# awslabs/dgl-ke

Hardware: AMD Instinct MI355X
Metric: positive edges/sec (whole node) (higher is better)
Workload: dtype f32

## Files before the change

dgl-ke_amd/csrc/kge_common.hpp:

```cpp
#pragma once
#include <hip/hip_runtime.h>
#include <stdint.h>
#include "../../include/kge_hip.h"

#define KGE_WAVE 64
#define KGE_BLOCK 256
#define KGE_WAVES_PER_BLOCK (KGE_BLOCK / KGE_WAVE)

typedef float f32x4 __attribute__((ext_vector_type(4)));
#define MFMA16(a, b, c) __builtin_amdgcn_mfma_f32_16x16x4f32((a), (b), (c), 0, 0, 0)

#ifdef KGE_TIMELINE
#define KGE_TL_PER_KERNEL 8192
static __device__ unsigned long long *kge_tl_buf = nullptr;
__device__ __forceinline__ void kge_tl_mark(int kid, int n) {
    asm volatile("s_waitcnt vmcnt(0) lgkmcnt(0)" ::: "memory");
    const int wid = (int)(blockIdx.x * (blockDim.x >> 6) + (threadIdx.x >> 6));
    if ((threadIdx.x & 63) == 0 && kge_tl_buf && wid < KGE_TL_PER_KERNEL)
        kge_tl_buf[((size_t)kid * KGE_TL_PER_KERNEL + wid) * 8 + 4 + n] = wall_clock64();
}
struct KgeTlScope {
    unsigned long long t0; int kid; int wid;
    __device__ __forceinline__ KgeTlScope(int kid_, int wid_) : kid(kid_), wid(wid_) { t0 = wall_clock64(); }
    __device__ __forceinline__ void mark(int n) { kge_tl_mark(kid, n); }
// ... 152 lines not shown
__device__ __forceinline__ float sgnf(float x) { return (x > 0.f) ? 1.f : ((x < 0.f) ? -1.f : 0.f); }

__device__ __forceinline__ float reg_grad3(float x, float coef) { return 3.f * coef * x * fabsf(x); }
__device__ __forceinline__ float reg_val3(float x) { const float ax = fabsf(x); return ax * ax * ax; }
__device__ __forceinline__ float reg_grad(float x, float coef, int q) {
    if (__builtin_constant_p(q) && q == 3) return reg_grad3(x, coef);
    const float ax = fabsf(x);
    const float pw = __builtin_amdgcn_exp2f((float)(q - 1) * __builtin_amdgcn_logf(ax));
    return ax > 0.f ? copysignf(coef * (float)q * pw, x) : 0.f;
}
__device__ __forceinline__ float reg_val(float x, int q) {
    if (__builtin_constant_p(q) && q == 3) return reg_val3(x);
    const float ax = fabsf(x);
    return ax > 0.f ? __builtin_amdgcn_exp2f((float)q * __builtin_amdgcn_logf(ax)) : 0.f;
}

__device__ __forceinline__ float reg_acc(float rv, float x, int q) {
    if (__builtin_constant_p(q) && q == 3) { const float ax = fabsf(x); return fmaf(ax * ax, ax, rv); }
    return rv + reg_val(x, q);
}

__device__ __forceinline__ float sigmoidf_(float x) {
    if (x >= 0.f) { return 1.f / (1.f + expf(-x)); }
    const float e = expf(x);
    return e / (1.f + e);
}
__device__ __forceinline__ float neg_logsigmoid(float z) {
    return fmaxf(-z, 0.f) + log1pf(expf(-fabsf(z)));
}

constexpr bool is_complex_model(int m) { return m == KGE_COMPLEX || m == KGE_ROTATE || m == KGE_SIMPLE; }
#define KGE_SIMPLE_CLAMP 20.f

__device__ __forceinline__ float fast_sigmoid(float x) { return __frcp_rn(1.f + __expf(-x)); }
__device__ __forceinline__ float fast_neg_logsigmoid(float z) {
    return fmaxf(-z, 0.f) + __logf(1.f + __expf(-fabsf(z)));
}
__device__ __forceinline__ void criterion_fast(int genre, float s, float label, float margin,
                                               float &val, float &dval) {
    if (genre == KGE_LOSS_HINGE) {
        const float v = margin - label * s;
        val = v < 0.f ? 0.f : v;
        dval = v < 0.f ? 0.f : -label;
    } else if (genre == KGE_LOSS_BCE) {
        val = label * fast_neg_logsigmoid(s) + (1.f - label) * fast_neg_logsigmoid(-s);
        dval = fast_sigmoid(s) - label;
    } else {
        const float z = label * s;
        val = fast_neg_logsigmoid(z);
        dval = -label * fast_sigmoid(-z);
    }
}

__device__ __forceinline__ void criterion(int genre, float s, float label, float margin,
                                          float &val, float &dval) {
    criterion_fast(genre, s, label, margin, val, dval);
}

__device__ __forceinline__ float mean_edge_weight(const float *w, int B, int lane, float pre = 0.f) {
    if (!w) return 1.f;
    if (pre > 0.f) return pre;
    float s = 0.f;
    for (int j = lane; j < B; j += KGE_WAVE) s += w[j];
    return wave_sum(s) / (float)B;
}

__device__ __forceinline__ int xcd_remap(int b, int nb) {
    const int q = nb >> 3, r = nb & 7, x = b & 7, k = b >> 3;
    return (x < r ? x * (q + 1) : r * (q + 1) + (x - r) * q) + k;
}

}

struct EdgeSrc {
    const float *hbase; const int64_t *hidx;
    const float *tbase; const int64_t *tidx;
    const float *rbase; const int64_t *ridx;
    kge::ShardMap em, rm;
};

struct LossParams {
    int genre, adv, pairwise;
    float adv_temp, margin;
// ... 60 lines not shown
    for (int r = 0; r < 8; ++r) pv[r] = *reinterpret_cast<const float4 *>(a.GNp + (int64_t)(r < nrw ? r : nrw - 1) * stride + 4 * t);
    float4 acc = pv[0];
#pragma unroll
    for (int r = 1; r < 8; ++r)
        if (r < nrw) { acc.x += pv[r].x; acc.y += pv[r].y; acc.z += pv[r].z; acc.w += pv[r].w; }
    for (int r = 8; r < nrw; ++r) {
        const float4 v = *reinterpret_cast<const float4 *>(a.GNp + r * stride + 4 * t);
        acc.x += v.x; acc.y += v.y; acc.z += v.z; acc.w += v.w;
    }
    if (a.reg_coef > 0.f && a.reg_norm > 0) {
        const int64_t j = (4 * t) / a.d_e;
        const int k = (int)((4 * t) % a.d_e);
        const float4 x = *reinterpret_cast<const float4 *>(kge::row_ptr(a.nbase, a.nidx, j, a.d_e) + k);
        acc.x += kge::reg_grad(x.x, a.reg_coef, a.reg_norm); acc.y += kge::reg_grad(x.y, a.reg_coef, a.reg_norm);
        acc.z += kge::reg_grad(x.z, a.reg_coef, a.reg_norm); acc.w += kge::reg_grad(x.w, a.reg_coef, a.reg_norm);
    }
    { kge::Pack<4> o; o.v[0] = acc.x; o.v[1] = acc.y; o.v[2] = acc.z; o.v[3] = acc.w; KGE_ST_NEXT<4>(a.GN + 4 * t, o); }
}

struct LossArgs {
    int B, N, genre, adv, pairwise;
    float adv_temp, margin;
    const float *pos, *neg, *w;
    float w_mean;
    float *dpos, *dneg;
    float *row_pos, *row_neg;
    float *acc;
    int l2_scale; float gamma;
    int l2_raw, l2_chunk; const float *asq, *bsq;
    float clampv;
    float *neg_copy;
    int skip_pos;
    int diag_chunk;
};

struct UpdateArgs {
    int model_d_e, d_r, UE, UR, reg_norm;
    float lr, eps, reg_coef;
    float *ent, *ent_state, *rel, *rel_state;
    kge::ShardMap em, rm;
    const int64_t *ue_id; const int32_t *ue_pos_ptr, *ue_pos_adj, *ue_neg_ptr, *ue_neg_slot;
    const int64_t *ur_id; const int32_t *ur_ptr, *ur_edge;
    const int32_t *ue_rec, *ur_rec;
    const int32_t *counts_dev;
    const float *GH, *GT, *GN, *GR;
    int transe_fast, neg_head; const float *P, *GA;
    const float *Q;
    float *reg_ent, *reg_rel;
    float *acc;
    float *g0, *gs0, *g1, *gs1, *gr, *gsr;
    int emit_ent, emit_rel;
    int emit_by_id;
    const int32_t *msg_rows;
    int msg_cap, msg_capT;
    int ld_e, ld_r;
    int32_t *rid;
    int ld_gs_e, ld_gs_r;
    int dry;
    const float *Hs, *Ts, *Rs;
    const float *Ns;
    int nd_chunk, nd_Ns, nd_Np;
    const float *GNp; int gn_parts; int64_t gn_stride; float gn_reg_coef; int gn_reg_norm;
    int ga_parts; int64_t ga_stride;
};
__device__ __forceinline__ int64_t gn_row(const UpdateArgs &a, int slot) {
    return a.nd_chunk ? (int64_t)(slot / a.nd_Ns) * a.nd_Np + a.nd_chunk + slot % a.nd_Ns : (int64_t)slot;
}
// ... 194 lines not shown
```

dgl-ke_amd/csrc/kge_loss_body.hpp:

```cpp
#pragma once
#include "kge_common.hpp"
#include "kge_update_body.hpp"

__device__ __forceinline__ void loss_args_lean(LossArgs &a) {
    a.genre = KGE_LOSS_LOGSIGMOID; a.pairwise = 0; a.skip_pos = 1; a.clampv = 0.f; a.neg_copy = nullptr;
    a.row_pos = nullptr; a.row_neg = nullptr; a.diag_chunk = 0;
}

template <int NPER>
__device__ __forceinline__ void loss_row_regs(const LossArgs &a, int64_t i, float (&nv)[NPER], float w, float p, int lane,
                                              int slot2) {
    using namespace kge;
    const int N = a.N;
    float *dn = a.dneg + i * (int64_t)N;
    float *cp = a.neg_copy ? a.neg_copy + i * (int64_t)N : nullptr;
    const int jd = a.diag_chunk > 0 ? (int)(i % a.diag_chunk) : -1;
    const float invB = 1.f / (float)a.B;
    const int slot = (int)(i & (KGE_ACC_SLOTS - 1));
    if (a.pairwise) {
        const float sc = w / ((float)a.B * (float)N);
        float lsum = 0.f, dsum = 0.f;
#pragma unroll
        for (int u = 0; u < NPER; ++u) {
            const int j = lane + 64 * u;
            if (j < N) {
                float val, dv;
                criterion_fast(a.genre, p - nv[u], 1.f, a.margin, val, dv);
                lsum += val * sc;
                const float dd = dv * sc;
                dsum += dd;
                if (cp) cp[j] = nv[u];
                float g = -dd;
                if (a.l2_scale) { const float d = a.gamma - nv[u]; g = d > 1e-15f ? g / d : 0.f; }
                if (a.clampv > 0.f && fabsf(nv[u]) >= a.clampv) g = 0.f;
                dn[j] = j == jd ? 0.f : g;
            }
        }
        lsum = wave_sum(lsum);
        dsum = wave_sum(dsum);
        if (lane == 0) {
            a.dpos[i] = (a.clampv > 0.f && fabsf(p) >= a.clampv) ? 0.f : dsum;
            if (a.row_pos) { a.row_pos[i] = 0.f; a.row_neg[i] = lsum; }
            if (a.acc) acc_add(&a.acc[2 * KGE_ACC_SLOTS + slot2], lsum, a.B <= KGE_ACC_SLOTS);
        }
        return;
    }
    float plw = 0.f;
    if (!a.skip_pos) {
        const float wm = mean_edge_weight(a.w, a.B, lane, a.w_mean);
        if (lane == 0) {
            float pl, dpl;
            criterion(a.genre, p, 1.f, a.margin, pl, dpl);
            a.dpos[i] = (a.clampv > 0.f && fabsf(p) >= a.clampv) ? 0.f : dpl * wm * 0.5f * invB;
            plw = pl * wm * invB;
            if (a.row_pos) a.row_pos[i] = plw;
        }
    }
    const float neg_label = a.genre == KGE_LOSS_BCE ? 0.f : -1.f;
    float mx = -INFINITY, Z = 1.f;
    float ex[NPER];
    if (a.adv) {
#pragma unroll
        for (int u = 0; u < NPER; ++u) if (lane + 64 * u < N) mx = fmaxf(mx, nv[u] * a.adv_temp);
        mx = wave_max(mx);
        float z = 0.f;
#pragma unroll
        for (int u = 0; u < NPER; ++u) {
            ex[u] = (lane + 64 * u < N) ? __expf(nv[u] * a.adv_temp - mx) : 0.f;
            z += ex[u];
        }
        Z = wave_sum(z);
    }
    const float invZ = 1.f / Z, invN = 1.f / (float)N;
    float acc = 0.f;
#pragma unroll
    for (int u = 0; u < NPER; ++u) {
        const int j = lane + 64 * u;
        if (j < N) {
            float nl, dnl;
            criterion_fast(a.genre, nv[u], neg_label, a.margin, nl, dnl);
            const float A = a.adv ? ex[u] * invZ : invN;
            acc += A * nl * w;
            float g = dnl * w * A * 0.5f * invB;
            if (cp) cp[j] = nv[u];
            if (a.l2_scale) { const float d = a.gamma - nv[u]; g = d > 1e-15f ? g / d : 0.f; }
            if (a.clampv > 0.f && fabsf(nv[u]) >= a.clampv) g = 0.f;
            dn[j] = j == jd ? 0.f : g;
        }
    }
    acc = wave_sum(acc) * invB;
    if (lane == 0) {
        if (a.row_neg) a.row_neg[i] = acc;
        if (a.acc) {
            const bool uq = a.B <= KGE_ACC_SLOTS;
            if (!a.skip_pos) acc_add(&a.acc[0 * KGE_ACC_SLOTS + slot], plw, uq);
            acc_add(&a.acc[1 * KGE_ACC_SLOTS + slot], acc, uq);
            acc_add(&a.acc[2 * KGE_ACC_SLOTS + slot2], 0.5f * (plw + acc), uq);
        }
    }
}
```

dgl-ke_amd/csrc/kge_neg_gemm.hip:

```cpp
#include "kge_common.hpp"
#include "kge_update_body.hpp"
#include "kge_edge_fwd_body.hpp"
#include "kge_sampler_tail.hpp"
#include "kge_loss_body.hpp"

using namespace kge;
KGE_TL_DEFINE(gemm)

#define KGE_PIN_ACC(x, y) do { asm volatile("" : "+a"(x), "+a"(y) :: "memory"); __builtin_amdgcn_sched_barrier(0); } while (0)
#define KGE_ORDER() do { asm volatile("" ::: "memory"); __builtin_amdgcn_sched_barrier(0); } while (0)

bool neg_mfma_supported(int model, int d_e, int N) {
    (void)N;
    if (model != KGE_TRANSE_L2 && model != KGE_DISTMULT && model != KGE_COMPLEX && model != KGE_SIMPLE &&
        model != KGE_RESCAL) return false;
    return d_e % 4 == 0;
}

bool neg_gemm_fused_loss_supported(int chunk, int N) { return N <= 256 && chunk <= 768; }

__device__ __forceinline__ float4 ldg4(const float *p) { return *reinterpret_cast<const float4 *>(p); }
__device__ __forceinline__ float4 zero4() { return make_float4(0.f, 0.f, 0.f, 0.f); }
__device__ __forceinline__ float sq4(const float4 &v) { return v.x * v.x + v.y * v.y + v.z * v.z + v.w * v.w; }

// ... 243 lines not shown
        float4 av[1], rv[1], bv[NB][1];
        av[0] = zero4(); rv[0] = zero4();
#pragma unroll
        for (int n = 0; n < NB; ++n) bv[n][0] = zero4();
        if (kfull * 16 + q * 4 < D) {
            av[0] = ldg4(Ap + kfull * 16);
            if (AM) rv[0] = ldg4(Rp + kfull * 16);
#pragma unroll
            for (int n = 0; n < NB; ++n) bv[n][0] = ldg4(Bp[n] + kfull * 16);
        }
        WF_MMA1(av, rv, bv, 0)
    }
#undef WF_LOAD
#undef WF_AFRAG
#undef WF_MMA1
#undef WF_MMA
#undef WF_MMA_G
#undef WF_PIN
#pragma unroll
    for (int n = 0; n < NB; ++n) {
        const int j = (jg * NB + n) * 16 + m;
#pragma unroll
        for (int r = 0; r < 4; ++r) {
            const int i = it * 16 + q * 4 + r;
            if (j < a.N && i < a.chunk) a.S[((int64_t)c * a.chunk + i) * a.N + j] = acc[n][0][r] + acc[n][1][r];
        }
    }
}

static inline int fwd_lds_stride(int D) { return ((D + 15) & ~15) + 4; }
static inline size_t fwd_lds_bytes(int D) { return (size_t)16 * fwd_lds_stride(D) * sizeof(float); }
static inline size_t fwd_lds_bytes_lf(int D) { return fwd_lds_bytes(D) + 32 * sizeof(float); }

template <int AM, bool LF = false, bool LLEAN = false>
__device__ __forceinline__ void neg_fwd_gemm_ldsa_body(const GemmArgs &a, int ti, int tj, int bid, int nblk, float *As,
                                                       const LossArgs *lap = nullptr, int *tickets = nullptr) {
    const int lane = threadIdx.x & 63, wv = threadIdx.x >> 6;
    const int tjg = (tj + 3) >> 2;
    int jg, sidx;
    const int nfull = (tj & 3) ? tjg - 1 : tjg, nheavy = a.C * ti * nfull;
    if (bid < nheavy) { const int L = xcd_remap(bid, nheavy); jg = L % nfull; sidx = L / nfull; }
    else { sidx = xcd_remap(bid - nheavy, nblk - nheavy); jg = tjg - 1; }
    const int it = sidx % ti, c = sidx / ti;
    const int jt = min(jg * 4 + wv, tj - 1);
    const bool tile_ok = jg * 4 + wv < tj;
    const int D = a.D, KP = ((D + 15) & ~15) + 4, n4 = D >> 2;
    const int m = lane & 15, q = lane >> 4;
    const int arow = threadIdx.x >> 4, ac = threadIdx.x & 15;
    const int64_t ie = (int64_t)c * a.chunk + min(it * 16 + arow, a.chunk - 1);
    const int64_t jl = (int64_t)c * a.N + min(jt * 16 + m, a.N - 1);
    const int64_t xid = a.xidx[ie], rid = a.ridx[ie];
    const int64_t jraw = *(a.nidx ? a.nidx + jl : a.xidx);
    const float *Xs = a.xbase + xid * D, *Rs = a.rbase + rid * D;
    const float *Bp = a.nbase + (a.nidx ? jraw : jl) * D + q * 4;
    float *Adst = As + arow * KP;
    const float *Ap = As + m * KP + q * 4;
    const float asg = a.asign;
    const int kfull = D >> 4;
    f32x4 acc0 = {0.f, 0.f, 0.f, 0.f}, acc1 = {0.f, 0.f, 0.f, 0.f};
    float4 a0[FU], b0[FU], a1[FU], b1[FU];
    float4 xv[8], rv[8];
    float asq_t = 0.f, bs0 = 0.f, bs1 = 0.f;
    if constexpr (AM == 3) {
        const int hd = D >> 1, h4 = hd >> 2;
        for (int c0 = 0; c0 < h4; c0 += 16 * 4) {
#pragma unroll
// ... 119 lines not shown
    } else {
        float bsq = 0.f;
        if constexpr (AM == 1) {
            bsq = bs0 + bs1;
            bsq += __shfl_xor(bsq, 16);
            bsq += __shfl_xor(bsq, 32);
        }
#pragma unroll
        for (int r = 0; r < 4; ++r) {
            const int i = it * 16 + q * 4 + r;
            float x = acc0[r] + acc1[r];
            if constexpr (AM == 1) x = a.gamma - sqrtf(fmaxf(fmaf(-2.f, x, Aq[q * 4 + r] + bsq), 1e-30f));
            if (j < a.N && i < a.chunk)
                __hip_atomic_store(a.S + ((int64_t)c * a.chunk + i) * a.N + j, x, __ATOMIC_RELAXED, __HIP_MEMORY_SCOPE_AGENT);
        }
    }
    }
    if constexpr (LF) {
        asm volatile("s_waitcnt vmcnt(0)" ::: "memory");
        __syncthreads();
        int *lastw = reinterpret_cast<int *>(Aq + 16);
        if (threadIdx.x == 0) {
            int *tk = tickets + (c * ti + it);
            const int old = __hip_atomic_fetch_add(tk, 1, __ATOMIC_RELAXED, __HIP_MEMORY_SCOPE_AGENT);
            const int last = old == tjg - 1;
            if (last) __hip_atomic_store(tk, 0, __ATOMIC_RELAXED, __HIP_MEMORY_SCOPE_AGENT);
            else if (old < 0 || old >= tjg) __builtin_trap();
            *lastw = last;
        }
        __syncthreads();
        if (!*lastw) return;
        LossArgs la = *lap;
        if constexpr (LLEAN) loss_args_lean(la);
        constexpr int NPER = 4;
        const int N = la.N;
        const int row0 = it * 16 + wv * 4;
        float nv[4][NPER];
#pragma unroll
        for (int r = 0; r < 4; ++r) {
            const int64_t gi = (int64_t)c * a.chunk + min(row0 + r, a.chunk - 1);
#pragma unroll
            for (int u = 0; u < NPER; ++u)
                nv[r][u] = __hip_atomic_load(a.S + gi * N + min(lane + 64 * u, N - 1), __ATOMIC_RELAXED, __HIP_MEMORY_SCOPE_AGENT);
        }
        float wr[4];
#pragma unroll
        for (int r = 0; r < 4; ++r) wr[r] = la.w ? la.w[(int64_t)c * a.chunk + min(row0 + r, a.chunk - 1)] : 1.f;
#pragma unroll
        for (int r = 0; r < 4; ++r) {
            if (row0 + r < a.chunk) {
                const int64_t gi = (int64_t)c * a.chunk + row0 + r;
#pragma unroll
                for (int u = 0; u < NPER; ++u) if (lane + 64 * u >= N) nv[r][u] = 0.f;
                loss_row_regs<NPER>(la, gi, nv[r], wr[r], 0.f, lane, (int)((gi + la.B) & (KGE_ACC_SLOTS - 1)));
            }
        }
    }
}

#define KGE_FWD_NB 1
template <bool L2, int AM, int MODEL, bool LEAN, bool LDSA>
__global__ __launch_bounds__(KGE_BLOCK) void neg_fwd_edge_kernel(const int64_t *xidx, const int64_t *ridx, const int64_t *nidx, int nbG, int nbM,
                                                                 int ti, int tj, int C, int chunk, int N, int D, GemmArgs a_in,
                                                                 EdgeFwdArgs e, SmpTail st) {
    extern __shared__ __attribute__((aligned(16))) float smem[];
    if ((int)blockIdx.x < nbG) {
        KGE_TL(1);
        GemmArgs a = a_in;
        a.xidx = xidx; a.ridx = ridx; a.nidx = nidx; a.C = C; a.chunk = chunk; a.N = N; a.D = D;
        if constexpr (LDSA) neg_fwd_gemm_ldsa_body<AM>(a, ti, tj, (int)blockIdx.x, nbG, smem);
        else if constexpr (KGE_FWD_NB == 1) neg_fwd_gemm_body<L2, false, AM>(a, ti, tj, (int)blockIdx.x, nbG);
        else neg_fwd_gemm_wide_body<AM, KGE_FWD_NB>(a, ti, (tj + KGE_FWD_NB - 1) / KGE_FWD_NB, (int)blockIdx.x, nbG);
    } else if ((int)blockIdx.x < nbM) {
        KGE_TL(0);
        edge_fwd_body<MODEL, 4, LEAN>(e, (int)blockIdx.x - nbG);
    } else {
        sampler_tail_p1(st, (int)blockIdx.x - nbM);
    }
}

template <int AM, int MODEL, bool LEAN>
__global__ __launch_bounds__(KGE_BLOCK) void neg_fwd_loss_edge_kernel(GemmArgs a, int ti, int tj, int nbG, EdgeFwdArgs e, LossArgs la,
                                                                      int *tickets) {
    extern __shared__ __attribute__((aligned(16))) float smem[];
    if ((int)blockIdx.x < nbG) {
        KGE_TL(1);
        neg_fwd_gemm_ldsa_body<AM, true, LEAN>(a, ti, tj, (int)blockIdx.x, nbG, smem, &la, tickets);
    } else {
        KGE_TL(0);
// ... 17 lines not shown
    EdgeFwdArgs ee = e;
    if (!negjob) ee.n_neg = 0;
    const int nbP = (int)((waves + KGE_WAVES_PER_BLOCK - 1) / KGE_WAVES_PER_BLOCK);
    const int ti = (a.chunk + 15) / 16, tj = (a.N + 15) / 16;
    const size_t lds = fwd_lds_bytes(a.D);
    const bool ldsa = lds <= 64 * 1024 && !a.lds_off;
    const int64_t ntiles = (int64_t)a.C * ti * ((tj + KGE_FWD_NB - 1) / KGE_FWD_NB);
    const int nbG = ldsa ? a.C * ti * ((tj + 3) / 4) : (int)((ntiles + KGE_WAVES_PER_BLOCK - 1) / KGE_WAVES_PER_BLOCK);
    const bool lean = e.lp.genre == KGE_LOSS_LOGSIGMOID && !e.row_pos && !e.Hc;
    const int nbM = nbG + nbP;
    const dim3 g(nbM + (st.phase ? ST_P1_WGS + (st.slot3 ? ST_P3_WGS : 0) : 0)), b(KGE_BLOCK);
#define KGE_FE_H a.xidx, a.ridx, a.nidx, nbG, nbM, ti, tj, a.C, a.chunk, a.N, a.D, a, ee, st
#define KGE_FE2(L2_, AM_, M_, LE_) do { if (ldsa) hipLaunchKernelGGL((neg_fwd_edge_kernel<L2_, AM_, M_, LE_, true>), g, b, lds, s, KGE_FE_H); \
                                        else hipLaunchKernelGGL((neg_fwd_edge_kernel<L2_, AM_, M_, LE_, false>), g, b, 0, s, KGE_FE_H); } while (0)
#define KGE_FE(L2_, AM_, M_) do { if (lean) KGE_FE2(L2_, AM_, M_, true); else KGE_FE2(L2_, AM_, M_, false); } while (0)
    if (a.model == KGE_COMPLEX) {
        if (!ldsa) return KGE_ERR_ARG;
        if (lean) hipLaunchKernelGGL((neg_fwd_edge_kernel<false, 3, KGE_COMPLEX, true, true>), g, b, lds, s, KGE_FE_H);
        else hipLaunchKernelGGL((neg_fwd_edge_kernel<false, 3, KGE_COMPLEX, false, true>), g, b, lds, s, KGE_FE_H);
    } else if (a.model == KGE_TRANSE_L2) KGE_FE(true, 1, KGE_TRANSE_L2);
    else KGE_FE(false, 2, KGE_DISTMULT);
#undef KGE_FE
#undef KGE_FE2
#undef KGE_FE_H
    return check_launch();
}

bool neg_fwd_loss_fold_supported(int model, int C, int chunk, int N, int d_e, int d_r) {
    if (!neg_fwd_gemm_with_edge_supported(model, d_e, d_r) || fwd_lds_bytes_lf(d_e) > 64 * 1024) return false;
    if (N > 256 || (N & 1) || (((int64_t)chunk * N) & 31)) return false;
    return (int64_t)C * ((chunk + 15) / 16) <= KGE_TICKET_INTS;
}

int launch_neg_fwd_gemm_with_edge_loss(const GemmArgs &a, const EdgeFwdArgs &e, const LossArgs &la, int *tickets, hipStream_t s) {
    if (a.C == 0 || a.PM || !a.xbase || !a.rbase || !a.xidx || !a.ridx || !tickets || a.lds_off) return KGE_ERR_ARG;
    if (!neg_fwd_loss_fold_supported(a.model, a.C, a.chunk, a.N, a.D, e.d_r) || e.model != a.model || e.d_e != a.D) return KGE_ERR_ARG;
    if (e.src.em.n || e.src.rm.n || e.nd_own || la.pairwise || !la.skip_pos || la.l2_raw || la.diag_chunk > 0 || la.neg != a.S ||
        la.dneg != a.S || la.N != a.N || la.B != a.C * a.chunk) return KGE_ERR_ARG;
    const bool negjob = e.bsq || e.Bn;
    const int64_t waves = (int64_t)e.B + (negjob ? e.n_neg : 0);
    EdgeFwdArgs ee = e;
    if (!negjob) ee.n_neg = 0;
    const int nbP = (int)((waves + KGE_WAVES_PER_BLOCK - 1) / KGE_WAVES_PER_BLOCK);
    const int ti = (a.chunk + 15) / 16, tj = (a.N + 15) / 16;
    const size_t lds = fwd_lds_bytes_lf(a.D);
    const int nbG = a.C * ti * ((tj + 3) / 4);
    const bool lean = e.lp.genre == KGE_LOSS_LOGSIGMOID && !e.row_pos && !e.Hc &&
                      la.genre == KGE_LOSS_LOGSIGMOID && la.clampv == 0.f && !la.neg_copy && !la.row_pos && !la.row_neg;
    const dim3 g(nbG + nbP), b(KGE_BLOCK);
#define KGE_FL(AM_, M_) do { if (lean) hipLaunchKernelGGL((neg_fwd_loss_edge_kernel<AM_, M_, true>), g, b, lds, s, a, ti, tj, nbG, ee, la, tickets); \
                             else hipLaunchKernelGGL((neg_fwd_loss_edge_kernel<AM_, M_, false>), g, b, lds, s, a, ti, tj, nbG, ee, la, tickets); } while (0)
    if (a.model == KGE_COMPLEX) KGE_FL(3, KGE_COMPLEX);
    else if (a.model == KGE_TRANSE_L2) KGE_FL(1, KGE_TRANSE_L2);
    else KGE_FL(2, KGE_DISTMULT);
#undef KGE_FL
    return check_launch();
}

int launch_neg_fwd_gemm(const GemmArgs &a, hipStream_t s) {
    const int ti = (a.chunk + 15) / 16, tj = (a.N + 15) / 16;
    const int64_t ntiles = (int64_t)a.C * ti * tj;
    if (ntiles == 0) return KGE_OK;
    const int nb = (int)((ntiles + KGE_WAVES_PER_BLOCK - 1) / KGE_WAVES_PER_BLOCK);
    const bool l2 = a.model == KGE_TRANSE_L2, st = a.PM != nullptr;
    const dim3 g(nb), b(KGE_BLOCK);
    if (l2 && st) hipLaunchKernelGGL((neg_fwd_gemm_kernel<true, true>), g, b, 0, s, a, ti, tj);
    else if (l2) hipLaunchKernelGGL((neg_fwd_gemm_kernel<true, false>), g, b, 0, s, a, ti, tj);
// ... 579 lines not shown
```

dgl-ke_amd/csrc/kge_rowwise.hip:

```cpp
#include "kge_common.hpp"
#include "kge_update_body.hpp"
#include "kge_sampler_tail.hpp"
#include "kge_edge_fwd_body.hpp"
#include "kge_loss_body.hpp"

using namespace kge;
KGE_TL_DEFINE(rowwise)

#define WAVE_ID() ((int64_t)blockIdx.x * KGE_WAVES_PER_BLOCK + (threadIdx.x >> 6))

static inline int blocks_for_waves(int64_t waves) {
    return (int)((waves + KGE_WAVES_PER_BLOCK - 1) / KGE_WAVES_PER_BLOCK);
}

template <int V>
__global__ __launch_bounds__(KGE_BLOCK) void gather_kernel(const float *__restrict__ table, int dim,
                                                           const int64_t *__restrict__ idx,
                                                           int64_t n, float *__restrict__ out) {
    const int64_t k = WAVE_ID();
    if (k >= n) return;
    const int lane = LANE();
    const float *src = table + idx[k] * (int64_t)dim;
    float *dst = out + k * (int64_t)dim;
    for (int it = lane; it < dim / V; it += 64) st<V>(dst + it * V, ld<V>(src + it * V));
// ... 470 lines not shown
        for (int j = lane; j < N; j += 64) mx = fmaxf(mx, (j == jd ? 0.f : n[j]) * a.adv_temp);
        mx = wave_max(mx);
        float z = 0.f;
        for (int j = lane; j < N; j += 64) z += expf((j == jd ? 0.f : n[j]) * a.adv_temp - mx);
        Z = wave_sum(z);
    }
    const float invZ = 1.f / Z, invN = 1.f / (float)N;
    float acc = 0.f;
    for (int j = lane; j < N; j += 64) {
        const float nv = j == jd ? 0.f : n[j];
        float nl, dnl;
        criterion(a.genre, nv, neg_label, a.margin, nl, dnl);
        const float A = a.adv ? expf(nv * a.adv_temp - mx) * invZ : invN;
        acc += A * nl * w;
        float g = dnl * w * A * 0.5f * invB;
        if (cp) cp[j] = nv;
        if (a.l2_scale) { const float d = a.gamma - nv; g = d > 1e-15f ? g / d : 0.f; }
        if (a.clampv > 0.f && fabsf(nv) >= a.clampv) g = 0.f;
        dn[j] = j == jd ? 0.f : g;
    }
    acc = wave_sum(acc) * invB;
    if (lane == 0) {
        if (a.row_neg) a.row_neg[i] = acc;
        if (a.acc) {
            const int slot = (int)(i & (KGE_ACC_SLOTS - 1));
            const bool uq = a.B <= KGE_ACC_SLOTS;
            if (!a.skip_pos) acc_add(&a.acc[0 * KGE_ACC_SLOTS + slot], plw, uq);
            acc_add(&a.acc[1 * KGE_ACC_SLOTS + slot], acc, uq);
            acc_add(&a.acc[2 * KGE_ACC_SLOTS + (int)((a.skip_pos ? i + a.B : i) & (KGE_ACC_SLOTS - 1))], 0.5f * (plw + acc), uq);
        }
    }
}

template <int NPER, bool LEAN, bool RAW>
__global__ __launch_bounds__(KGE_BLOCK) void loss_kernel_reg(const float *neg, const float *bsq, const float *asq, const float *pos,
                                                             const float *w_, int B_, int N_, int l2_chunk, LossArgs a_in) {
    KGE_TL(2);
    LossArgs a = a_in;
    a.neg = neg; a.bsq = bsq; a.asq = asq; a.pos = pos; a.w = w_; a.B = B_; a.N = N_; a.l2_chunk = l2_chunk;
    if constexpr (LEAN) loss_args_lean(a);
    const int64_t i = WAVE_ID();
    if (i >= a.B) return;
    const int lane = LANE();
    const int N = a.N;
    const float *n = a.neg + i * (int64_t)N;
    float nv[NPER];
    const int jd = a.diag_chunk > 0 ? (int)(i % a.diag_chunk) : -1;
#pragma unroll
    for (int u = 0; u < NPER; ++u) { const int j = lane + 64 * u; nv[u] = (j < N && j != jd) ? n[j] : 0.f; }
    float bq[RAW ? NPER : 1], asq_i = 0.f;
    if constexpr (RAW) {
        const float *bqp = a.bsq + (i / a.l2_chunk) * (int64_t)N;
#pragma unroll
        for (int u = 0; u < NPER; ++u) { const int j = lane + 64 * u; bq[u] = j < N ? bqp[j] : 0.f; }
        asq_i = a.asq[i];
    }
    const float w = a.w ? a.w[i] : 1.f;
    const float p = a.pos[i];
    if constexpr (RAW) {
#pragma unroll
        for (int u = 0; u < NPER; ++u) {
            const int j = lane + 64 * u;
            nv[u] = (j < N && j != jd) ? a.gamma - sqrtf(fmaxf(fmaf(-2.f, nv[u], asq_i + bq[u]), 1e-30f)) : 0.f;
        }
    }
    KGE_TL_MARK(0);
    loss_row_regs<NPER>(a, i, nv, w, p, lane, (int)((a.skip_pos ? i + a.B : i) & (KGE_ACC_SLOTS - 1)));
    KGE_TL_MARK(1);
}

int launch_loss(const LossArgs &a, hipStream_t s) {
    if (a.B == 0) return KGE_OK;
    const dim3 g(blocks_for_waves(a.B)), b(KGE_BLOCK);
    const bool lean = a.genre == KGE_LOSS_LOGSIGMOID && !a.pairwise && a.skip_pos && a.clampv == 0.f && !a.neg_copy &&
                      !a.row_pos && !a.row_neg && a.diag_chunk <= 0;
    if (a.l2_raw && (!a.asq || !a.bsq || a.l2_chunk <= 0)) return KGE_ERR_ARG;
#define KGE_LOSS_H a.neg, a.bsq, a.asq, a.pos, a.w, a.B, a.N, a.l2_chunk, a
#define KGE_LOSS(N) do { if (a.l2_raw) { if (lean) hipLaunchKernelGGL((loss_kernel_reg<N, true, true>), g, b, 0, s, KGE_LOSS_H); \
                                         else hipLaunchKernelGGL((loss_kernel_reg<N, false, true>), g, b, 0, s, KGE_LOSS_H); } \
                         else if (lean) hipLaunchKernelGGL((loss_kernel_reg<N, true, false>), g, b, 0, s, KGE_LOSS_H); \
                         else hipLaunchKernelGGL((loss_kernel_reg<N, false, false>), g, b, 0, s, KGE_LOSS_H); } while (0)
    if (a.N <= 64) KGE_LOSS(1);
    else if (a.N <= 128) KGE_LOSS(2);
    else if (a.N <= 256) KGE_LOSS(4);
    else if (a.N <= 512) KGE_LOSS(8);
    else hipLaunchKernelGGL(loss_kernel, g, b, 0, s, a);
#undef KGE_LOSS
#undef KGE_LOSS_H
    return check_launch();
}

__device__ float block_sum_det(const float *x, int n, float *sh) {
    float v = 0.f;
    if (x) for (int k = threadIdx.x; k < n; k += KGE_BLOCK) v += x[k];
    v = wave_sum(v);
    __syncthreads();
    if ((threadIdx.x & 63) == 0) sh[threadIdx.x >> 6] = v;
    __syncthreads();
    return sh[0] + sh[1] + sh[2] + sh[3];
}

__global__ __launch_bounds__(KGE_BLOCK) void finalize_kernel(FinalizeArgs a) {
    __shared__ float sh[KGE_WAVES_PER_BLOCK];
    const float lp = block_sum_det(a.row_pos, a.B, sh);
    const float ln = block_sum_det(a.row_neg, a.B, sh);
    const float re = block_sum_det(a.reg_ent, a.counts_dev ? a.counts_dev[0] : a.UE, sh);
    const float rr = block_sum_det(a.reg_rel, a.counts_dev ? a.counts_dev[1] : a.UR, sh);
    if (threadIdx.x == 0) {
        float o[4];
        if (a.pairwise) { o[0] = NAN; o[1] = NAN; o[2] = ln; }
        else { o[0] = lp; o[1] = ln; o[2] = 0.5f * (lp + ln); }
        o[3] = re + rr;
        if (a.loss4) for (int k = 0; k < 4; ++k) a.loss4[k] = o[k];
    }
}

__global__ __launch_bounds__(KGE_BLOCK) void reduce_acc_kernel(float *acc, float *out4, int zero_after) {
    __shared__ float sh[KGE_WAVES_PER_BLOCK];
// ... 465 lines not shown
```

Before: 34.37 million.

## Vectorize negative-loss row loads/stores and share sigmoid/log work in criterion

Loss rows are now loaded and stored as float4 packs when N is a multiple of four and pointers are 16-byte aligned, with a new column mapping. The loss body is restructured to compute criteria for all columns first, then softmax weighting with paired vector math, then scaling and a single store. The sigmoid and log-sigmoid are fused into one helper that shares an exp, a reciprocal and a log, and divisions are replaced with hardware rcp. The intent is fewer memory instructions and fewer transcendental ops in the per-row loss, at the cost of a layout change where each lane owns contiguous columns, and slightly lower precision from approximate rcp/log.

Result: faster. 35.43 million, median of 6 (+3.1%).

```diff
diff --git a/dgl-ke_amd/csrc/kge_common.hpp b/dgl-ke_amd/csrc/kge_common.hpp
--- a/dgl-ke_amd/csrc/kge_common.hpp
+++ b/dgl-ke_amd/csrc/kge_common.hpp
@@ -208,9 +208,15 @@
 constexpr bool is_complex_model(int m) { return m == KGE_COMPLEX || m == KGE_ROTATE || m == KGE_SIMPLE; }
 #define KGE_SIMPLE_CLAMP 20.f
 
-__device__ __forceinline__ float fast_sigmoid(float x) { return __frcp_rn(1.f + __expf(-x)); }
-__device__ __forceinline__ float fast_neg_logsigmoid(float z) {
-    return fmaxf(-z, 0.f) + __logf(1.f + __expf(-fabsf(z)));
+struct SoftSig { float lg, sig, nsig; };
+__device__ __forceinline__ SoftSig fast_soft_sig(float z) {
+    const float e = __expf(-fabsf(z)), t = 1.f + e;
+    const float r = __builtin_amdgcn_rcpf(t), er = e * r;
+    SoftSig o;
+    o.lg = __builtin_amdgcn_logf(t) * 0.6931471805599453f;
+    o.sig = z >= 0.f ? r : er;
+    o.nsig = z >= 0.f ? er : r;
+    return o;
 }
 __device__ __forceinline__ void criterion_fast(int genre, float s, float label, float margin,
                                                float &val, float &dval) {
@@ -219,12 +225,14 @@
         val = v < 0.f ? 0.f : v;
         dval = v < 0.f ? 0.f : -label;
     } else if (genre == KGE_LOSS_BCE) {
-        val = label * fast_neg_logsigmoid(s) + (1.f - label) * fast_neg_logsigmoid(-s);
-        dval = fast_sigmoid(s) - label;
+        const SoftSig q = fast_soft_sig(s);
+        val = label * (fmaxf(-s, 0.f) + q.lg) + (1.f - label) * (fmaxf(s, 0.f) + q.lg);
+        dval = q.sig - label;
     } else {
         const float z = label * s;
-        val = fast_neg_logsigmoid(z);
-        dval = -label * fast_sigmoid(-z);
+        const SoftSig q = fast_soft_sig(z);
+        val = fmaxf(-z, 0.f) + q.lg;
+        dval = -label * q.nsig;
     }
 }
 
@@ -351,7 +359,14 @@
     float *neg_copy;
     int skip_pos;
     int diag_chunk;
-};
+    float inv_B, inv_N;
+    int pk;
+};
+inline void loss_fill_host(LossArgs &a) {
+    a.inv_B = 1.f / (float)a.B; a.inv_N = 1.f / (float)a.N;
+    auto al = [](const void *p) { return (reinterpret_cast<uintptr_t>(p) & 15) == 0; };
+    a.pk = a.N > 0 && a.N % 4 == 0 && al(a.neg) && al(a.dneg) && al(a.neg_copy) && (!a.l2_raw || al(a.bsq));
+}
 
 struct UpdateArgs {
     int model_d_e, d_r, UE, UR, reg_norm;
diff --git a/dgl-ke_amd/csrc/kge_loss_body.hpp b/dgl-ke_amd/csrc/kge_loss_body.hpp
--- a/dgl-ke_amd/csrc/kge_loss_body.hpp
+++ b/dgl-ke_amd/csrc/kge_loss_body.hpp
@@ -7,35 +7,76 @@
     a.row_pos = nullptr; a.row_neg = nullptr; a.diag_chunk = 0;
 }
 
-template <int NPER>
+typedef float f32x2 __attribute__((ext_vector_type(2)));
+template <bool PK> __device__ __forceinline__ int loss_col(int lane, int u) {
+    return PK ? 4 * (lane + 64 * (u >> 2)) + (u & 3) : lane + 64 * u;
+}
+template <bool PK> __device__ __forceinline__ bool loss_live(int lane, int u, int N) {
+    return (PK ? 4 * (lane + 64 * (u >> 2)) : lane + 64 * u) < N;
+}
+template <bool PK> __device__ __forceinline__ int loss_ld_col(int lane, int u, int N) {
+    return PK ? 4 * min(lane + 64 * (u >> 2), (N >> 2) - 1) : min(lane + 64 * u, N - 1);
+}
+template <int NPER, bool PK>
+__device__ __forceinline__ void loss_row_load(const float *p, int lane, int N, float (&x)[NPER]) {
+    if constexpr (PK) {
+        static_assert(NPER % 4 == 0, "packs of four columns");
+#pragma unroll
+        for (int q = 0; q < NPER / 4; ++q) {
+            const f32x4 v = *reinterpret_cast<const f32x4 *>(p + loss_ld_col<true>(lane, 4 * q, N));
+            x[4 * q] = v.x; x[4 * q + 1] = v.y; x[4 * q + 2] = v.z; x[4 * q + 3] = v.w;
+        }
+    } else {
+#pragma unroll
+        for (int u = 0; u < NPER; ++u) x[u] = p[loss_ld_col<false>(lane, u, N)];
+    }
+}
+template <int NPER, bool PK>
+__device__ __forceinline__ void loss_row_store(float *p, int lane, int N, const float (&x)[NPER]) {
+    if constexpr (PK) {
+#pragma unroll
+        for (int q = 0; q < NPER / 4; ++q)
+            if (loss_live<true>(lane, 4 * q, N)) {
+                f32x4 v; v.x = x[4 * q]; v.y = x[4 * q + 1]; v.z = x[4 * q + 2]; v.w = x[4 * q + 3];
+                *reinterpret_cast<f32x4 *>(p + loss_col<true>(lane, 4 * q)) = v;
+            }
+    } else {
+#pragma unroll
+        for (int u = 0; u < NPER; ++u) if (loss_live<false>(lane, u, N)) p[loss_col<false>(lane, u)] = x[u];
+    }
+}
+
+template <int NPER, bool PK>
 __device__ __forceinline__ void loss_row_regs(const LossArgs &a, int64_t i, float (&nv)[NPER], float w, float p, int lane,
                                               int slot2) {
     using namespace kge;
     const int N = a.N;
     float *dn = a.dneg + i * (int64_t)N;
-    float *cp = a.neg_copy ? a.neg_copy + i * (int64_t)N : nullptr;
     const int jd = a.diag_chunk > 0 ? (int)(i % a.diag_chunk) : -1;
-    const float invB = 1.f / (float)a.B;
+    const float invB = a.inv_B;
     const int slot = (int)(i & (KGE_ACC_SLOTS - 1));
+    float g[NPER];
+    if (a.neg_copy) loss_row_store<NPER, PK>(a.neg_copy + i * (int64_t)N, lane, N, nv);
     if (a.pairwise) {
         const float sc = w / ((float)a.B * (float)N);
         float lsum = 0.f, dsum = 0.f;
 #pragma unroll
         for (int u = 0; u < NPER; ++u) {
-            const int j = lane + 64 * u;
-            if (j < N) {
-                float val, dv;
-                criterion_fast(a.genre, p - nv[u], 1.f, a.margin, val, dv);
-                lsum += val * sc;
-                const float dd = dv * sc;
-                dsum += dd;
-                if (cp) cp[j] = nv[u];
-                float g = -dd;
-                if (a.l2_scale) { const float d = a.gamma - nv[u]; g = d > 1e-15f ? g / d : 0.f; }
-                if (a.clampv > 0.f && fabsf(nv[u]) >= a.clampv) g = 0.f;
-                dn[j] = j == jd ? 0.f : g;
-            }
+            float val, dv;
+            criterion_fast(a.genre, p - nv[u], 1.f, a.margin, val, dv);
+            const bool live = loss_live<PK>(lane, u, N);
+            lsum += live ? val * sc : 0.f;
+            const float dd = dv * sc;
+            dsum += live ? dd : 0.f;
+            g[u] = -dd;
         }
+#pragma unroll
+        for (int u = 0; u < NPER; ++u) {
+            if (a.l2_scale) { const float d = a.gamma - nv[u]; g[u] = d > 1e-15f ? g[u] * __builtin_amdgcn_rcpf(d) : 0.f; }
+            if (a.clampv > 0.f && fabsf(nv[u]) >= a.clampv) g[u] = 0.f;
+            if (loss_col<PK>(lane, u) == jd) g[u] = 0.f;
+        }
+        loss_row_store<NPER, PK>(dn, lane, N, g);
         lsum = wave_sum(lsum);
         dsum = wave_sum(dsum);
         if (lane == 0) {
@@ -57,38 +98,89 @@
         }
     }
     const float neg_label = a.genre == KGE_LOSS_BCE ? 0.f : -1.f;
-    float mx = -INFINITY, Z = 1.f;
-    float ex[NPER];
+    float nl[NPER];
+#pragma unroll
+    for (int u = 0; u < NPER; ++u) criterion_fast(a.genre, nv[u], neg_label, a.margin, nl[u], g[u]);
+    constexpr int GS = PK ? 4 : 1;
+    constexpr int PW = PK ? 2 : 1;
+    float acc = 0.f, rs;
     if (a.adv) {
+        float mx = -INFINITY;
 #pragma unroll
-        for (int u = 0; u < NPER; ++u) if (lane + 64 * u < N) mx = fmaxf(mx, nv[u] * a.adv_temp);
+        for (int q = 0; q < NPER; q += GS) {
+            float m = nv[q] * a.adv_temp;
+#pragma unroll
+            for (int u = q + 1; u < q + GS; ++u) m = fmaxf(m, nv[u] * a.adv_temp);
+            mx = fmaxf(mx, loss_live<PK>(lane, q, N) ? m : -INFINITY);
+        }
         mx = wave_max(mx);
         float z = 0.f;
 #pragma unroll
-        for (int u = 0; u < NPER; ++u) {
-            ex[u] = (lane + 64 * u < N) ? __expf(nv[u] * a.adv_temp - mx) : 0.f;
-            z += ex[u];
+        for (int q = 0; q < NPER; q += GS) {
+            float zq = 0.f, aq = 0.f;
+#pragma unroll
+            for (int u = q; u < q + GS; u += PW) {
+                if constexpr (PW == 2) {
+                    const f32x2 sv = {nv[u], nv[u + 1]};
+                    const f32x2 t = sv * a.adv_temp - mx;
+                    const f32x2 ex = {__expf(t.x), __expf(t.y)};
+                    f32x2 gg = {g[u], g[u + 1]};
+                    gg *= ex;
+                    g[u] = gg.x; g[u + 1] = gg.y;
+                    zq += ex.x; zq += ex.y;
+                    aq = fmaf(ex.x, nl[u], aq); aq = fmaf(ex.y, nl[u + 1], aq);
+                } else {
+                    const float ex = __expf(nv[u] * a.adv_temp - mx);
+                    zq += ex;
+                    aq = fmaf(ex, nl[u], aq);
+                    g[u] *= ex;
+                }
+            }
+            const bool live = loss_live<PK>(lane, q, N);
+            z += live ? zq : 0.f;
+            acc += live ? aq : 0.f;
         }
-        Z = wave_sum(z);
+        z = wave_sum(z);
+        acc = wave_sum(acc);
+        rs = __builtin_amdgcn_rcpf(z);
+    } else {
+#pragma unroll
+        for (int q = 0; q < NPER; q += GS) {
+            float aq = 0.f;
+#pragma unroll
+            for (int u = q; u < q + GS; ++u) aq += nl[u];
+            acc += loss_live<PK>(lane, q, N) ? aq : 0.f;
+        }
+        acc = wave_sum(acc);
+        rs = a.inv_N;
     }
-    const float invZ = 1.f / Z, invN = 1.f / (float)N;
-    float acc = 0.f;
+    const float ws = w * rs;
+    acc = acc * ws * invB;
+    const float gs = ws * 0.5f * invB;
+#pragma unroll
+    for (int u = 0; u < NPER; u += PW) {
+        if constexpr (PW == 2) {
+            f32x2 gg = {g[u], g[u + 1]};
+            gg *= gs;
+            if (a.l2_scale) {
+                const f32x2 sv = {nv[u], nv[u + 1]};
+                const f32x2 d = a.gamma - sv;
+                const f32x2 r = {__builtin_amdgcn_rcpf(d.x), __builtin_amdgcn_rcpf(d.y)};
+                gg *= r;
+                gg.x = d.x > 1e-15f ? gg.x : 0.f; gg.y = d.y > 1e-15f ? gg.y : 0.f;
+            }
+            g[u] = gg.x; g[u + 1] = gg.y;
+        } else {
+            g[u] *= gs;
+            if (a.l2_scale) { const float d = a.gamma - nv[u]; g[u] = d > 1e-15f ? g[u] * __builtin_amdgcn_rcpf(d) : 0.f; }
+        }
+    }
 #pragma unroll
     for (int u = 0; u < NPER; ++u) {
-        const int j = lane + 64 * u;
-        if (j < N) {
-            float nl, dnl;
-            criterion_fast(a.genre, nv[u], neg_label, a.margin, nl, dnl);
-            const float A = a.adv ? ex[u] * invZ : invN;
-            acc += A * nl * w;
-            float g = dnl * w * A * 0.5f * invB;
-            if (cp) cp[j] = nv[u];
-            if (a.l2_scale) { const float d = a.gamma - nv[u]; g = d > 1e-15f ? g / d : 0.f; }
-            if (a.clampv > 0.f && fabsf(nv[u]) >= a.clampv) g = 0.f;
-            dn[j] = j == jd ? 0.f : g;
-        }
+        if (a.clampv > 0.f && fabsf(nv[u]) >= a.clampv) g[u] = 0.f;
+        if (loss_col<PK>(lane, u) == jd) g[u] = 0.f;
     }
-    acc = wave_sum(acc) * invB;
+    loss_row_store<NPER, PK>(dn, lane, N, g);
     if (lane == 0) {
         if (a.row_neg) a.row_neg[i] = acc;
         if (a.acc) {
diff --git a/dgl-ke_amd/csrc/kge_neg_gemm.hip b/dgl-ke_amd/csrc/kge_neg_gemm.hip
--- a/dgl-ke_amd/csrc/kge_neg_gemm.hip
+++ b/dgl-ke_amd/csrc/kge_neg_gemm.hip
@@ -299,6 +299,48 @@
 static inline size_t fwd_lds_bytes(int D) { return (size_t)16 * fwd_lds_stride(D) * sizeof(float); }
 static inline size_t fwd_lds_bytes_lf(int D) { return fwd_lds_bytes(D) + 32 * sizeof(float); }
 
+template <bool PK>
+__device__ __forceinline__ void lf_loss_rows(const GemmArgs &a, const LossArgs &la, int c, int row0, int lane) {
+    constexpr int NPER = 4;
+    const int N = la.N;
+    float nv[4][NPER], wr[4];
+#pragma unroll
+    for (int r = 0; r < 4; ++r) wr[r] = la.w ? la.w[(int64_t)c * a.chunk + min(row0 + r, a.chunk - 1)] : 1.f;
+    if constexpr (PK) {
+        const float *q[4];
+#pragma unroll
+        for (int r = 0; r < 4; ++r)
+            q[r] = a.S + ((int64_t)c * a.chunk + min(row0 + r, a.chunk - 1)) * N + loss_ld_col<true>(lane, 0, N);
+        f32x4 v0, v1, v2, v3;
+        asm volatile("global_load_dwordx4 %0, %4, off sc1\n\t"
+                     "global_load_dwordx4 %1, %5, off sc1\n\t"
+                     "global_load_dwordx4 %2, %6, off sc1\n\t"
+                     "global_load_dwordx4 %3, %7, off sc1\n\t"
+                     "s_waitcnt vmcnt(0)"
+                     : "=&v"(v0), "=&v"(v1), "=&v"(v2), "=&v"(v3) : "v"(q[0]), "v"(q[1]), "v"(q[2]), "v"(q[3]) : "memory");
+        const f32x4 v[4] = {v0, v1, v2, v3};
+#pragma unroll
+        for (int r = 0; r < 4; ++r) { nv[r][0] = v[r].x; nv[r][1] = v[r].y; nv[r][2] = v[r].z; nv[r][3] = v[r].w; }
+    } else {
+#pragma unroll
+        for (int r = 0; r < 4; ++r) {
+            const int64_t gi = (int64_t)c * a.chunk + min(row0 + r, a.chunk - 1);
+#pragma unroll
+            for (int u = 0; u < NPER; ++u)
+                nv[r][u] = __hip_atomic_load(a.S + gi * N + loss_ld_col<false>(lane, u, N), __ATOMIC_RELAXED, __HIP_MEMORY_SCOPE_AGENT);
+        }
+    }
+#pragma unroll
+    for (int r = 0; r < 4; ++r) {
+        if (row0 + r < a.chunk) {
+            const int64_t gi = (int64_t)c * a.chunk + row0 + r;
+#pragma unroll
+            for (int u = 0; u < NPER; ++u) if (!loss_live<PK>(lane, u, N)) nv[r][u] = 0.f;
+            loss_row_regs<NPER, PK>(la, gi, nv[r], wr[r], 0.f, lane, (int)((gi + la.B) & (KGE_ACC_SLOTS - 1)));
+        }
+    }
+}
+
 template <int AM, bool LF = false, bool LLEAN = false>
 __device__ __forceinline__ void neg_fwd_gemm_ldsa_body(const GemmArgs &a, int ti, int tj, int bid, int nblk, float *As,
                                                        const LossArgs *lap = nullptr, int *tickets = nullptr) {
@@ -484,29 +526,8 @@
         if (!*lastw) return;
         LossArgs la = *lap;
         if constexpr (LLEAN) loss_args_lean(la);
-        constexpr int NPER = 4;
-        const int N = la.N;
-        const int row0 = it * 16 + wv * 4;
-        float nv[4][NPER];
-#pragma unroll
-        for (int r = 0; r < 4; ++r) {
-            const int64_t gi = (int64_t)c * a.chunk + min(row0 + r, a.chunk - 1);
-#pragma unroll
-            for (int u = 0; u < NPER; ++u)
-                nv[r][u] = __hip_atomic_load(a.S + gi * N + min(lane + 64 * u, N - 1), __ATOMIC_RELAXED, __HIP_MEMORY_SCOPE_AGENT);
-        }
-        float wr[4];
-#pragma unroll
-        for (int r = 0; r < 4; ++r) wr[r] = la.w ? la.w[(int64_t)c * a.chunk + min(row0 + r, a.chunk - 1)] : 1.f;
-#pragma unroll
-        for (int r = 0; r < 4; ++r) {
-            if (row0 + r < a.chunk) {
-                const int64_t gi = (int64_t)c * a.chunk + row0 + r;
-#pragma unroll
-                for (int u = 0; u < NPER; ++u) if (lane + 64 * u >= N) nv[r][u] = 0.f;
-                loss_row_regs<NPER>(la, gi, nv[r], wr[r], 0.f, lane, (int)((gi + la.B) & (KGE_ACC_SLOTS - 1)));
-            }
-        }
+        if (la.pk) lf_loss_rows<true>(a, la, c, it * 16 + wv * 4, lane);
+        else lf_loss_rows<false>(a, la, c, it * 16 + wv * 4, lane);
     }
 }
 
@@ -590,7 +611,9 @@
     return (int64_t)C * ((chunk + 15) / 16) <= KGE_TICKET_INTS;
 }
 
-int launch_neg_fwd_gemm_with_edge_loss(const GemmArgs &a, const EdgeFwdArgs &e, const LossArgs &la, int *tickets, hipStream_t s) {
+int launch_neg_fwd_gemm_with_edge_loss(const GemmArgs &a, const EdgeFwdArgs &e, const LossArgs &la_, int *tickets, hipStream_t s) {
+    LossArgs la = la_;
+    loss_fill_host(la);
     if (a.C == 0 || a.PM || !a.xbase || !a.rbase || !a.xidx || !a.ridx || !tickets || a.lds_off) return KGE_ERR_ARG;
     if (!neg_fwd_loss_fold_supported(a.model, a.C, a.chunk, a.N, a.D, e.d_r) || e.model != a.model || e.d_e != a.D) return KGE_ERR_ARG;
     if (e.src.em.n || e.src.rm.n || e.nd_own || la.pairwise || !la.skip_pos || la.l2_raw || la.diag_chunk > 0 || la.neg != a.S ||
diff --git a/dgl-ke_amd/csrc/kge_rowwise.hip b/dgl-ke_amd/csrc/kge_rowwise.hip
--- a/dgl-ke_amd/csrc/kge_rowwise.hip
+++ b/dgl-ke_amd/csrc/kge_rowwise.hip
@@ -526,58 +526,60 @@
     }
 }
 
-template <int NPER, bool LEAN, bool RAW>
+template <int NPER, bool LEAN, bool RAW, bool PK>
 __global__ __launch_bounds__(KGE_BLOCK) void loss_kernel_reg(const float *neg, const float *bsq, const float *asq, const float *pos,
                                                              const float *w_, int B_, int N_, int l2_chunk, LossArgs a_in) {
     KGE_TL(2);
     LossArgs a = a_in;
     a.neg = neg; a.bsq = bsq; a.asq = asq; a.pos = pos; a.w = w_; a.B = B_; a.N = N_; a.l2_chunk = l2_chunk;
     if constexpr (LEAN) loss_args_lean(a);
-    const int64_t i = WAVE_ID();
-    if (i >= a.B) return;
+    if constexpr (RAW) a.l2_scale = 1;
+    const int i32 = (int)blockIdx.x * KGE_WAVES_PER_BLOCK + __builtin_amdgcn_readfirstlane((int)(threadIdx.x >> 6));
+    if (i32 >= a.B) return;
+    const int64_t i = i32;
     const int lane = LANE();
     const int N = a.N;
-    const float *n = a.neg + i * (int64_t)N;
     float nv[NPER];
     const int jd = a.diag_chunk > 0 ? (int)(i % a.diag_chunk) : -1;
-#pragma unroll
-    for (int u = 0; u < NPER; ++u) { const int j = lane + 64 * u; nv[u] = (j < N && j != jd) ? n[j] : 0.f; }
+    loss_row_load<NPER, PK>(a.neg + i * (int64_t)N, lane, N, nv);
     float bq[RAW ? NPER : 1], asq_i = 0.f;
     if constexpr (RAW) {
-        const float *bqp = a.bsq + (i / a.l2_chunk) * (int64_t)N;
-#pragma unroll
-        for (int u = 0; u < NPER; ++u) { const int j = lane + 64 * u; bq[u] = j < N ? bqp[j] : 0.f; }
+        loss_row_load<NPER, PK>(a.bsq + (int64_t)((unsigned)i32 / (unsigned)a.l2_chunk) * N, lane, N, bq);
         asq_i = a.asq[i];
     }
     const float w = a.w ? a.w[i] : 1.f;
     const float p = a.pos[i];
-    if constexpr (RAW) {
-#pragma unroll
-        for (int u = 0; u < NPER; ++u) {
-            const int j = lane + 64 * u;
-            nv[u] = (j < N && j != jd) ? a.gamma - sqrtf(fmaxf(fmaf(-2.f, nv[u], asq_i + bq[u]), 1e-30f)) : 0.f;
-        }
+#pragma unroll
+    for (int u = 0; u < NPER; ++u) {
+        if constexpr (RAW) nv[u] = a.gamma - sqrtf(fmaxf(fmaf(-2.f, nv[u], asq_i + bq[u]), 1e-30f));
+        if (!loss_live<PK>(lane, u, N) || loss_col<PK>(lane, u) == jd) nv[u] = 0.f;
     }
     KGE_TL_MARK(0);
-    loss_row_regs<NPER>(a, i, nv, w, p, lane, (int)((a.skip_pos ? i + a.B : i) & (KGE_ACC_SLOTS - 1)));
+    loss_row_regs<NPER, PK>(a, i, nv, w, p, lane, (int)((a.skip_pos ? i + a.B : i) & (KGE_ACC_SLOTS - 1)));
     KGE_TL_MARK(1);
 }
 
-int launch_loss(const LossArgs &a, hipStream_t s) {
-    if (a.B == 0) return KGE_OK;
+int launch_loss(const LossArgs &a_, hipStream_t s) {
+    if (a_.B == 0) return KGE_OK;
+    if (a_.N <= 0) return KGE_ERR_ARG;
+    LossArgs a = a_;
+    loss_fill_host(a);
     const dim3 g(blocks_for_waves(a.B)), b(KGE_BLOCK);
     const bool lean = a.genre == KGE_LOSS_LOGSIGMOID && !a.pairwise && a.skip_pos && a.clampv == 0.f && !a.neg_copy &&
                       !a.row_pos && !a.row_neg && a.diag_chunk <= 0;
-    if (a.l2_raw && (!a.asq || !a.bsq || a.l2_chunk <= 0)) return KGE_ERR_ARG;
+    if (a.l2_raw && (!a.asq || !a.bsq || a.l2_chunk <= 0 || !a.l2_scale)) return KGE_ERR_ARG;
+    const bool pk = a.pk != 0;
 #define KGE_LOSS_H a.neg, a.bsq, a.asq, a.pos, a.w, a.B, a.N, a.l2_chunk, a
-#define KGE_LOSS(N) do { if (a.l2_raw) { if (lean) hipLaunchKernelGGL((loss_kernel_reg<N, true, true>), g, b, 0, s, KGE_LOSS_H); \
-                                         else hipLaunchKernelGGL((loss_kernel_reg<N, false, true>), g, b, 0, s, KGE_LOSS_H); } \
-                         else if (lean) hipLaunchKernelGGL((loss_kernel_reg<N, true, false>), g, b, 0, s, KGE_LOSS_H); \
-                         else hipLaunchKernelGGL((loss_kernel_reg<N, false, false>), g, b, 0, s, KGE_LOSS_H); } while (0)
-    if (a.N <= 64) KGE_LOSS(1);
-    else if (a.N <= 128) KGE_LOSS(2);
-    else if (a.N <= 256) KGE_LOSS(4);
-    else if (a.N <= 512) KGE_LOSS(8);
+#define KGE_LOSS(N, PK) do { if (a.l2_raw) { if (lean) hipLaunchKernelGGL((loss_kernel_reg<N, true, true, PK>), g, b, 0, s, KGE_LOSS_H); \
+                                             else hipLaunchKernelGGL((loss_kernel_reg<N, false, true, PK>), g, b, 0, s, KGE_LOSS_H); } \
+                             else if (lean) hipLaunchKernelGGL((loss_kernel_reg<N, true, false, PK>), g, b, 0, s, KGE_LOSS_H); \
+                             else hipLaunchKernelGGL((loss_kernel_reg<N, false, false, PK>), g, b, 0, s, KGE_LOSS_H); } while (0)
+    if (pk && a.N <= 256) KGE_LOSS(4, true);
+    else if (pk && a.N <= 512) KGE_LOSS(8, true);
+    else if (a.N <= 64) KGE_LOSS(1, false);
+    else if (a.N <= 128) KGE_LOSS(2, false);
+    else if (a.N <= 256) KGE_LOSS(4, false);
+    else if (a.N <= 512) KGE_LOSS(8, false);
     else hipLaunchKernelGGL(loss_kernel, g, b, 0, s, a);
 #undef KGE_LOSS
 #undef KGE_LOSS_H
```
